# OpenRL-Lab/openrl

Measured on NVIDIA H100. Metric: env-steps/sec (collect+update), CartPole-v1 PPO, higher is better.
Workload: dtype f32 (nets, losses, Adam; the three 64x64 GEMM groups of the update run as split-fp16 wgmma MMAs with fp32 accumulation = fp32-class accuracy, the mode the 1e-4 parity tests run in), f64 (CartPole state)

## Files before the change

### include/openrl_b200.h

```cpp
#ifndef OPENRL_B200_H
#define OPENRL_B200_H

#include <stdint.h>

#ifdef __cplusplus
extern "C" {
#endif

#define ORL_ABI_VERSION 1

#define ORL_ERR_BAD_ARG 10001
#define ORL_ERR_UNSUPPORTED 10002

int orl_abi_version(void);
const char* orl_last_error(void);
int orl_device_sm_count(int* sm_count_out);

#define ORL_GAE_USE_GAE 1
#define ORL_GAE_PROPER_TIME_LIMITS 2
#define ORL_GAE_DENORM 4
#define ORL_GAE_NSTATS 8
#define ORL_GS_ADV_SUM 0
#define ORL_GS_ADV_SQSUM 1
#define ORL_GS_COUNT 2
// ... 49 lines not shown
    const float* exp_noise;
    uint64_t rng_seed;
    uint64_t rng_step_base;
    uint64_t* rng_counter;
    double* env_f64;
    uint64_t* env_u64;
    int32_t* env_i32;
    const int32_t* env_table;
    float* ep_return;
    int32_t* ep_length;
    double* episode_stats;
    int32_t head_kind;
    int32_t rng_row_offset;
} OrlRolloutArgs;
int orl_rollout(const OrlRolloutArgs* args, void* stream);

int orl_critic_values(const float* critic_params, int obs_dim, int activation_id,
                      const float* obs, float* values, long long rows, void* stream);

int orl_host_insert(const float* staged, int n_envs, int n_agents, int obs_dim, float* policy_obs_next, float* rewards,
                    float* masks_next, float* active_masks_next, void* stream);

int orl_policy_eval(const float* policy_params, int obs_dim, int n_actions, int activation_id, int head_kind,
                    const float* obs, const float* actions, const float* action_masks, float* log_probs,
                    float* entropy, long long rows, void* stream);


#define ORL_PPO_HUBER 1
#define ORL_PPO_CLIP_VALUE 2
#define ORL_PPO_VALUE_ACTIVE_MASKS 4
// ... 152 lines not shown
```

### openrl_b200/csrc/orl_fwd_tc.cu

```cuda
#include <algorithm>
#include <cstdlib>
#include <map>
#include <mutex>

#include "orl_envstep.cuh"
#include "orl_tc16.cuh"

namespace {
using namespace orl;
using namespace orl::tc;

constexpr int F_M = 128, F_NT = 256, FCW = 32;
constexpr uint32_t FPANEL_W = H * 16;
constexpr int S_LD = 68;
template <int M1, int MS>
struct FwdLayout {
    static constexpr uint32_t PANEL = M1 * 16, R1H = 0, R1L = 8 * PANEL, WH = 16 * PANEL, WL = WH + 8 * FPANEL_W, S = WL + 8 * FPANEL_W,
                              SMALL = S + MS * S_LD * 4;
};
using FLay = FwdLayout<F_M, F_M>;
constexpr uint32_t FPANEL = FLay::PANEL;
constexpr uint32_t F_SMALL_FLOATS = 8 * H + H + H + MAX_OUT * H + MAX_OUT;
constexpr uint32_t F_XCH_FLOATS = 2 * F_M * 2 + 2 * F_M * 8 + F_M * 8;
constexpr uint32_t F_SMEM = FLay::SMALL + 4 * (F_SMALL_FLOATS + F_XCH_FLOATS);

#define F_FOR_OUT(j) _Pragma("unroll") for (int j = 0; j < NOUT; ++j) if (NOUT != 8 || j < n)
#define F_ROWGROUP_SYNC()                                                      \
    do {                                                                       \
        switch (warp & 3) {                                                    \
            case 0: asm volatile("bar.sync 1, 64;" ::: "memory"); break;       \
            case 1: asm volatile("bar.sync 2, 64;" ::: "memory"); break;       \
            case 2: asm volatile("bar.sync 3, 64;" ::: "memory"); break;       \
            default: asm volatile("bar.sync 4, 64;" ::: "memory"); break;      \
        }                                                                      \
    } while (0)

template <int ACT>
__device__ __forceinline__ float f_act(float z, int activation_id) { return ACT == 1 ? fmaxf(z, 0.f) : act_fwd(z, activation_id); }

struct FwdCtx {
    uint8_t *R1h, *R1l;
    float *S, *w1t, *b1s, *b3f, *whf, *bhf, *xs, *xh, *xst;
    uint32_t aR1h, aR1l, aWh, aWl;
};

template <typename L = FLay>
__device__ __forceinline__ FwdCtx fwd_setup(uint8_t* smem, const float* __restrict__ params, int d, int n) {
    const int tid = threadIdx.x, nt = blockDim.x;
    FwdCtx c;
    c.R1h = smem + L::R1H; c.R1l = smem + L::R1L;
    uint8_t* Wh = smem + L::WH; uint8_t* Wl = smem + L::WL;
    c.S = reinterpret_cast<float*>(smem + L::S);
    c.w1t = reinterpret_cast<float*>(smem + L::SMALL);
    c.b1s = c.w1t + 8 * H; c.b3f = c.b1s + H; c.whf = c.b3f + H; c.bhf = c.whf + MAX_OUT * H;
    c.xs = c.bhf + MAX_OUT; c.xh = c.xs + 2 * F_M * 2; c.xst = c.xh + 2 * F_M * 8;
    const NetOffsets po = net_offsets(d, n);
    for (int i = tid; i < 8 * H; i += nt) { const int k = i / H, j = i % H; c.w1t[i] = (k < d) ? params[po.w1 + j * d + k] : 0.f; }
    for (int i = tid; i < H; i += nt) c.b1s[i] = params[po.b1 + i];
    for (int i = tid; i < H * 8; i += nt) {
        const int pnl = i / H, j = i % H;
        float w8[8];
#pragma unroll
        for (int c = 0; c < 8; ++c) w8[c] = params[po.w3 + j * H + 8 * pnl + c] * params[po.g1 + 8 * pnl + c];
        const uint32_t off = (uint32_t)pnl * FPANEL_W + j * 16;
        split_store8(Wh + off, Wl + off, w8, 1.0f);
    }
    for (int i = tid; i < MAX_OUT * H; i += nt) { const int j = i / H, k = i % H; c.whf[i] = (j < n) ? params[po.wh + j * H + k] * params[po.g3 + k] : 0.f; }
    for (int j = tid; j < H; j += nt) {
        float s = params[po.b3 + j];
        for (int k = 0; k < H; ++k) s = fmaf(params[po.w3 + j * H + k], params[po.be1 + k], s);
        c.b3f[j] = s;
    }
    for (int j = tid; j < MAX_OUT; j += nt) {
        float s = 0.f;
        if (j < n) { s = params[po.bh + j]; for (int k = 0; k < H; ++k) s = fmaf(params[po.wh + j * H + k], params[po.be3 + k], s); }
        c.bhf[j] = s;
    }
    fence_proxy_async();
    __syncthreads();
    c.aR1h = smem_u32(c.R1h); c.aR1l = smem_u32(c.R1l); c.aWh = smem_u32(Wh); c.aWl = smem_u32(Wl);
    return c;
}

template <int NOUT, int ACT, typename Overlap>
__device__ __forceinline__ void fwd_tile(const FwdCtx& c, const float (&x)[8], int d, int n, int activation_id,
                                         float (&out)[MAX_OUT], Overlap&& overlap) {
    const int tid = threadIdx.x, warp = tid >> 5, row = tid & 127, half = tid >> 7, cb = FCW * half;
    float n1[FCW];
#pragma unroll
    for (int q4 = 0; q4 < FCW; q4 += 4) {
        const float4 b = *reinterpret_cast<const float4*>(c.b1s + cb + q4);
        n1[q4] = b.x; n1[q4 + 1] = b.y; n1[q4 + 2] = b.z; n1[q4 + 3] = b.w;
    }
#pragma unroll
    for (int k = 0; k < 8; ++k) {
        if (k < d) {
#pragma unroll
            for (int q4 = 0; q4 < FCW; q4 += 4) {
                const float4 wv = *reinterpret_cast<const float4*>(c.w1t + k * H + cb + q4);
                n1[q4] = fmaf(x[k], wv.x, n1[q4]); n1[q4 + 1] = fmaf(x[k], wv.y, n1[q4 + 1]);
                n1[q4 + 2] = fmaf(x[k], wv.z, n1[q4 + 2]); n1[q4 + 3] = fmaf(x[k], wv.w, n1[q4 + 3]);
            }
        }
    }
    float s = 0.f, sq = 0.f;
#pragma unroll
    for (int i = 0; i < FCW; ++i) { n1[i] = f_act<ACT>(n1[i], activation_id); s += n1[i]; sq = fmaf(n1[i], n1[i], sq); }
    {
        *reinterpret_cast<float2*>(c.xs + (half * F_M + row) * 2) = make_float2(s, sq);
        F_ROWGROUP_SYNC();
        const float2 o = *reinterpret_cast<const float2*>(c.xs + ((half ^ 1) * F_M + row) * 2);
        s += o.x; sq += o.y;
    }
    const float mu1 = s * (1.f / H);
    const float rstd1 = 1.0f / sqrtf(fmaxf(sq * (1.f / H) - mu1 * mu1, 0.f) + LN_EPS);
#pragma unroll
    for (int i = 0; i < FCW; ++i) n1[i] = (n1[i] - mu1) * rstd1;
#pragma unroll
    for (int q8 = 0; q8 < FCW; q8 += 8) {
        const uint32_t off = (uint32_t)((cb + q8) >> 3) * FPANEL + row * 16;
        split_store8(c.R1h + off, c.R1l + off, n1 + q8, 1.0f);
    }
    fence_proxy_async();
    __syncthreads();
    {
        const uint64_t dK_A = desc_const(FPANEL, 128), dK_W = desc_const(FPANEL_W, 128);
        float z[32];
#pragma unroll
        for (int i = 0; i < 32; ++i) z[i] = 0.f;
        wgmma_fence();
#pragma unroll
        for (int pass = 0; pass < 3; ++pass) {
            const uint32_t aa = (pass == 0 ? c.aR1l : c.aR1h) + half * 64 * 16, bb = pass == 1 ? c.aWl : c.aWh;
#pragma unroll
            for (int kk = 0; kk < 4; ++kk)
                wgmma_f16_n64<0, 0>(z, desc_at(dK_A, aa + 2 * kk * FPANEL), desc_at(dK_W, bb + 2 * kk * FPANEL_W), (pass | kk) > 0);
        }
        wgmma_commit();
        overlap();
        wgmma_wait<0>();
        frag_store<64>(z, c.S + half * 64 * S_LD, S_LD);
    }
    __syncthreads();
    float n3[FCW];
#pragma unroll
    for (int q4 = 0; q4 < FCW; q4 += 4) {
        const float4 v = *reinterpret_cast<const float4*>(c.S + row * S_LD + cb + q4);
        n3[q4] = v.x; n3[q4 + 1] = v.y; n3[q4 + 2] = v.z; n3[q4 + 3] = v.w;
    }
    float s3 = 0.f, q3 = 0.f;
#pragma unroll
    for (int i = 0; i < FCW; ++i) { n3[i] += c.b3f[cb + i]; s3 += n3[i]; q3 = fmaf(n3[i], n3[i], q3); }
    {
        __syncwarp();
        *reinterpret_cast<float2*>(c.xs + (half * F_M + row) * 2) = make_float2(s3, q3);
        F_ROWGROUP_SYNC();
        const float2 o = *reinterpret_cast<const float2*>(c.xs + ((half ^ 1) * F_M + row) * 2);
        s3 += o.x; q3 += o.y;
    }
    const float mu3 = s3 * (1.f / H);
    const float rstd3 = 1.0f / sqrtf(fmaxf(q3 * (1.f / H) - mu3 * mu3, 0.f) + LN_EPS);
#pragma unroll
    for (int j = 0; j < MAX_OUT; ++j) out[j] = 0.f;
#pragma unroll
    for (int q4 = 0; q4 < FCW; q4 += 4) {
#pragma unroll
        for (int i = 0; i < 4; ++i) n3[q4 + i] = (n3[q4 + i] - mu3) * rstd3;
        F_FOR_OUT(j) {
            const float4 wv = *reinterpret_cast<const float4*>(c.whf + j * H + cb + q4);
            out[j] = fmaf(n3[q4], wv.x, fmaf(n3[q4 + 1], wv.y, fmaf(n3[q4 + 2], wv.z, fmaf(n3[q4 + 3], wv.w, out[j]))));
        }
    }
    {
        F_FOR_OUT(j) c.xh[(j * 2 + half) * F_M + row] = out[j];
        F_ROWGROUP_SYNC();
        F_FOR_OUT(j) {
            const float p0 = c.xh[(j * 2 + 0) * F_M + row], p1 = c.xh[(j * 2 + 1) * F_M + row];
            out[j] = (p0 + p1) + c.bhf[j];
        }
    }
}

template <int ACT>
__global__ void __launch_bounds__(F_NT, 2) critic_values_tc_kernel(const float* __restrict__ params, int d, int activation_id,
                                                                   const float* __restrict__ obs, float* __restrict__ values,
                                                                   long long rows) {
    extern __shared__ __align__(1024) uint8_t smem_f[];
    const FwdCtx c = fwd_setup(smem_f, params, d, 1);
    const int tid = threadIdx.x, warp = tid >> 5, row = tid & 127, half = tid >> 7;
    const long long n_tiles = (rows + F_M - 1) / F_M;
    for (long long tile = blockIdx.x; tile < n_tiles; tile += gridDim.x) {
        const long long r = tile * F_M + row;
        float x[8];
#pragma unroll
        for (int k = 0; k < 8; ++k) x[k] = (r < rows && k < d) ? obs[r * d + k] : 0.f;
        float out[MAX_OUT];
        fwd_tile<1, ACT>(c, x, d, 1, activation_id, out, [] {});
        if (half == 0 && r < rows) values[r] = out[0];
        F_ROWGROUP_SYNC();
    }
}

template <int ACT>
__global__ void __launch_bounds__(F_NT, 1) rollout_tc_kernel(const OrlRolloutArgs a) {
    extern __shared__ __align__(1024) uint8_t smem_f[];
    constexpr int NOUT = 5;
    const int N = a.n_envs, B = N, d = a.obs_dim, n = NOUT;
    const FwdCtx c = fwd_setup(smem_f, a.policy_params, d, n);
    const int tid = threadIdx.x, warp = tid >> 5, row = tid & 127, half = tid >> 7;
    const int e = blockIdx.x * F_M + row;
    const bool valid = e < N;
    const uint64_t rng_base = a.rng_step_base + (a.rng_counter ? *a.rng_counter : 0ull);
    float x[8];
#pragma unroll
    for (int k = 0; k < 8; ++k) x[k] = (valid && k < d) ? a.policy_obs[((size_t)a.t_begin * B + e) * d + k] : 0.f;
    {
        for (int t = a.t_begin; t < a.t_end; ++t) {
            float logit[MAX_OUT];
            float q[MAX_OUT];
            const size_t grow = (size_t)t * B + (valid ? e : 0);
            fwd_tile<NOUT, ACT>(c, x, d, n, a.activation_id, logit, [&] {
                if (half == 0 && valid && !a.deterministic)
                    action_noise(a.exp_noise, grow, n, a.rng_seed, rng_base + (uint64_t)t, (uint32_t)(e + a.rng_row_offset), q);
            });
            if (half == 0 && valid) {
                float lp;
                const int act = sample_action(logit, n, a.action_masks ? a.action_masks + grow * n : nullptr, a.deterministic != 0,
                                              [&](float (&qs)[MAX_OUT]) { for (int j = 0; j < MAX_OUT; ++j) qs[j] = q[j]; }, lp);
                a.actions[grow] = (float)act;
                a.action_log_probs[grow] = lp;
                EnvPtrs E{a.env_f64, a.env_u64, a.env_i32, a.env_table, a.env_table_len, a.rng_seed,
                          a.ep_return, a.ep_length, a.episode_stats, a.rng_row_offset};
                float ob[4], fin[4], reward; bool done;
                env_step_single(E, ORL_ENV_GRIDWORLD, e, N, act, ob, reward, done, fin);
                const size_t o1 = (size_t)(t + 1) * B + e;
                *reinterpret_cast<float4*>(a.policy_obs + o1 * 4) = make_float4(ob[0], ob[1], ob[2], ob[3]);
// ... 1 lines not shown
                a.masks[o1] = done ? 0.f : 1.f;
                a.active_masks[o1] = 1.f;
                *reinterpret_cast<float4*>(c.xst + row * 8) = make_float4(ob[0], ob[1], ob[2], ob[3]);
            }
            F_ROWGROUP_SYNC();
            if (valid) {
                const float4 o = *reinterpret_cast<const float4*>(c.xst + row * 8);
                x[0] = o.x; x[1] = o.y; x[2] = o.z; x[3] = o.w;
            }
        }
    }
}


constexpr int QCW = 16, RW_M = 64;
struct RowsCfg {
    static constexpr int R = 32, FWD = 4 * R, NT = 6 * R;
    static constexpr int MIN_CTAS = 3;
    using L = FwdLayout<RW_M, R>;
    static constexpr uint32_t XCH = L::SMALL + 4 * F_SMALL_FLOATS;
    static constexpr uint32_t XCH_F64 = XCH + 4 * (2 * MAX_OUT * R + 2 * R + 4 * R);
    static constexpr uint32_t SMEM = XCH_F64 + 8 * (2 * 2 * 4 * R + 2 * 4 * R);
    static_assert(XCH_F64 % 8 == 0, "f64 exchange area must be 8-byte aligned");
};

#define RW_FWD_SYNC() asm volatile("bar.sync 1, %0;" ::"n"(C::FWD) : "memory")
#define RW_PUBLISH_SYNC() asm volatile("bar.sync 2, %0;" ::"n"(C::NT) : "memory")

template <int ACT>
__global__ void __launch_bounds__(RowsCfg::NT, RowsCfg::MIN_CTAS) rollout_cartpole_rows_kernel(const OrlRolloutArgs a) {
    using C = RowsCfg;
    constexpr int R = C::R, NOUT = 2;
    extern __shared__ __align__(1024) uint8_t smem_f[];
    const int N = a.n_envs, B = N, n = NOUT;
    const int tid = threadIdx.x;
    for (int i = tid; i < 16 * (RW_M - R); i += C::NT) {
        const int p = i / (RW_M - R), r = R + i % (RW_M - R);
        *reinterpret_cast<uint4*>(smem_f + C::L::R1H + p * C::L::PANEL + r * 16) = make_uint4(0u, 0u, 0u, 0u);
    }
    const FwdCtx c = fwd_setup<typename C::L>(smem_f, a.policy_params, 4, n);
    float* qn = reinterpret_cast<float*>(smem_f + C::XCH);
    int* act_slot = reinterpret_cast<int*>(qn + 2 * MAX_OUT * R);
    int* termf = act_slot + 2 * R;
    double* cand = reinterpret_cast<double*>(smem_f + C::XCH_F64);
    double* srs = cand + 2 * 2 * 4 * R;
    const uint64_t rng_base = a.rng_step_base + (a.rng_counter ? *a.rng_counter : 0ull);
    uint32_t it = 0;
    if (tid >= C::FWD) {
        const int my_act = (tid - C::FWD) / R, row = (tid - C::FWD) % R;
        const int e = blockIdx.x * R + row;
        const bool valid = e < N;
        int elapsed = valid ? a.env_i32[e] : 0;
        double s[4] = {0, 0, 0, 0};
        Pcg64 g; g.state = 0; g.inc = 0;
        if (valid) {
#pragma unroll
            for (int k = 0; k < 4; ++k) s[k] = a.env_f64[(size_t)k * N + e];
            if (my_act == 0) g = pcg_load(a.env_u64, e, N);
        }
        const bool draw = my_act == 1 && valid && !a.deterministic;
        if (draw) {
            float q[MAX_OUT];
            action_noise(a.exp_noise, (size_t)a.t_begin * B + e, n, a.rng_seed, rng_base + (uint64_t)a.t_begin, (uint32_t)(e + a.rng_row_offset), q);
// ... 101 lines not shown
#pragma unroll
                    for (int kk = 0; kk < 4; ++kk)
#pragma unroll
                        for (int b = 0; b < 2; ++b)
                            wgmma_f16_n32<0, 0>(z[b], desc_at(dK_A, aa + 2 * kk * C::L::PANEL),
                                                desc_at(dK_W, bb + (nb0 + b) * 32 * 16 + 2 * kk * FPANEL_W), (pass | kk) > 0);
                }
                wgmma_commit();
                wgmma_wait<0>();
                if (16 * (warp & 3) < R) {
#pragma unroll
                    for (int b = 0; b < 2; ++b) frag_store<32>(z[b], c.S + 32 * (nb0 + b), S_LD);
                }
            }
            RW_FWD_SYNC();
            float n3[QCW];
#pragma unroll
            for (int q4 = 0; q4 < QCW; q4 += 4) {
                const float4 v = *reinterpret_cast<const float4*>(c.S + row * S_LD + cb + q4);
                n3[q4] = v.x; n3[q4 + 1] = v.y; n3[q4 + 2] = v.z; n3[q4 + 3] = v.w;
            }
            float s3 = 0.f, q3 = 0.f;
#pragma unroll
            for (int i = 0; i < QCW; ++i) { n3[i] += c.b3f[cb + i]; s3 += n3[i]; q3 = fmaf(n3[i], n3[i], q3); }
            {
                float ts = 0.f, tq = 0.f;
#pragma unroll
                for (int p = 0; p < 4; ++p) { ts += __shfl_sync(0xffffffffu, s3, qbase + p); tq += __shfl_sync(0xffffffffu, q3, qbase + p); }
                s3 = ts; q3 = tq;
            }
// ... 46 lines not shown
            if (qd == 0 && valid) {
                ret += 1.0f; len += 1;
                if (done) {
                    atomicAdd(a.episode_stats + 0, (double)ret);
                    atomicAdd(a.episode_stats + 1, (double)len);
                    atomicAdd(a.episode_stats + 2, 1.0);
                    ret = 0.f; len = 0;
                }
                const size_t o1 = (size_t)(t + 1) * B + e;
                *reinterpret_cast<float4*>(a.policy_obs + o1 * 4) = make_float4(x[0], x[1], x[2], x[3]);
                a.rewards[grow] = 1.0f;
                a.masks[o1] = done ? 0.f : 1.f;
                a.active_masks[o1] = 1.f;
            }
        }
        if (valid && qd == 0) { a.ep_return[e] = ret; a.ep_length[e] = len; }
    }
}
#undef RW_FWD_SYNC
#undef RW_PUBLISH_SYNC

template <typename K>
int prepare_kernel(K kern, uint32_t smem_bytes = F_SMEM) {
    static std::mutex mu;
    static std::map<const void*, bool> done;
    std::lock_guard<std::mutex> lock(mu);
    const void* key = reinterpret_cast<const void*>(kern);
    if (!done.count(key)) {
        int e = check_cuda(cudaFuncSetAttribute(kern, cudaFuncAttributeMaxDynamicSharedMemorySize, (int)smem_bytes), "cudaFuncSetAttribute(fwd_tc)");
        if (e) return e;
        done[key] = true;
    }
    return 0;
}

// ... 7 lines not shown
}

int launch_critic_values_tc(const float* params, int d, int activation_id, const float* obs, float* values, long long rows, cudaStream_t st) {
    const long long n_tiles = (rows + F_M - 1) / F_M;
    const int grid = (int)std::min<long long>(n_tiles, 2LL * sm_count());
    if (activation_id == 1) {
        if (int e = prepare_kernel(critic_values_tc_kernel<1>)) return e;
        critic_values_tc_kernel<1><<<grid, F_NT, F_SMEM, st>>>(params, d, activation_id, obs, values, rows);
    } else {
        if (int e = prepare_kernel(critic_values_tc_kernel<-1>)) return e;
        critic_values_tc_kernel<-1><<<grid, F_NT, F_SMEM, st>>>(params, d, activation_id, obs, values, rows);
    }
    return check_cuda(cudaGetLastError(), "critic_values_tc_kernel");
}

bool rollout_tc_eligible(const OrlRolloutArgs& a) {
    return fwd_tc_enabled() && (a.env_kind == ORL_ENV_CARTPOLE || a.env_kind == ORL_ENV_GRIDWORLD) && a.n_agents == 1 && a.obs_dim == 4 &&
           a.head_kind == ORL_HEAD_CATEGORICAL && (reinterpret_cast<uintptr_t>(a.policy_obs) & 15) == 0;
}

int launch_rollout_tc(const OrlRolloutArgs& a, cudaStream_t st) {
    const bool relu = a.activation_id == 1;
    if (a.env_kind == ORL_ENV_CARTPOLE) {
        const auto kern = relu ? rollout_cartpole_rows_kernel<1> : rollout_cartpole_rows_kernel<-1>;
        if (int e = prepare_kernel(kern, RowsCfg::SMEM)) return e;
        kern<<<(a.n_envs + RowsCfg::R - 1) / RowsCfg::R, RowsCfg::NT, RowsCfg::SMEM, st>>>(a);
        return check_cuda(cudaGetLastError(), "rollout_cartpole_rows_kernel");
    }
    const auto kern = relu ? rollout_tc_kernel<1> : rollout_tc_kernel<-1>;
    if (int e = prepare_kernel(kern)) return e;
    kern<<<(a.n_envs + F_M - 1) / F_M, F_NT, F_SMEM, st>>>(a);
    return check_cuda(cudaGetLastError(), "rollout_tc_kernel");
}

}
```

### openrl_b200/csrc/orl_rollout.cu

```cuda
#include "orl_envstep.cuh"

namespace {
using namespace orl;

constexpr int R_NT = 128;


__global__ void env_step_mpe_kernel(int N, EnvPtrs E, const float* __restrict__ actions, float* __restrict__ obs_out,
                                    float* __restrict__ critic_obs_out, float* __restrict__ rewards_out,
                                    float* __restrict__ dones_out) {
    const int e = blockIdx.x * blockDim.x + threadIdx.x;
    if (e >= N) return;
    const int acts[3] = {(int)actions[e * 3], (int)actions[e * 3 + 1], (int)actions[e * 3 + 2]};
    float ob[3][18], reward; bool done;
    env_step_mpe(E, e, N, acts, ob, reward, done);
    for (int ag = 0; ag < 3; ++ag) {
        for (int k = 0; k < 18; ++k) {
            obs_out[((size_t)e * 3 + ag) * 18 + k] = ob[ag][k];
            if (critic_obs_out) for (int dst = 0; dst < 3; ++dst) critic_obs_out[((size_t)e * 3 + dst) * 54 + ag * 18 + k] = ob[ag][k];
        }
        rewards_out[e * 3 + ag] = reward;
        dones_out[e * 3 + ag] = done ? 1.f : 0.f;
    }
}
// ... 301 lines not shown
                for (int j = 0; j < MAX_OUT; ++j) if (j < n) ent -= pr[j] * nl[j];
                logp_out[g] = lp;
                entropy_out[g] = ent;
            }
        }
        __syncthreads();
    }
}

}

namespace orl {
bool fwd_tc_enabled();
bool rollout_tc_eligible(const OrlRolloutArgs& a);
int launch_rollout_tc(const OrlRolloutArgs& a, cudaStream_t st);
int launch_critic_values_tc(const float* params, int d, int activation_id, const float* obs, float* values, long long rows, cudaStream_t st);
}

extern "C" int orl_env_reset(int env_kind, int n_envs, int n_agents, double* env_f64, uint64_t* env_u64,
                             int32_t* env_i32, const int32_t* env_table, int env_table_len, uint64_t rng_seed,
                             float* policy_obs_out, float* critic_obs_out, void* stream) {
    ORL_CHECK_ARG(n_envs > 0 && n_agents > 0, "n_envs/n_agents");
    ORL_CHECK_ARG(policy_obs_out, "policy_obs_out");
    if (env_kind == ORL_ENV_CARTPOLE) ORL_CHECK_ARG(env_f64 && env_u64 && env_i32 && n_agents == 1, "cartpole state");
    else if (env_kind == ORL_ENV_GRIDWORLD) ORL_CHECK_ARG(env_i32 && n_agents == 1, "gridworld state");
    else if (env_kind == ORL_ENV_MPE_SPREAD) ORL_CHECK_ARG(env_f64 && env_u64 && env_i32 && n_agents == 3, "simple_spread state");
    else { orl::set_last_error("orl_env_reset: unsupported env_kind %d", env_kind); return ORL_ERR_UNSUPPORTED; }
    cudaStream_t st = reinterpret_cast<cudaStream_t>(stream);
    env_reset_kernel<<<(n_envs + 127) / 128, 128, 0, st>>>(env_kind, n_envs, env_f64, env_u64, env_i32, env_table,
                                                          env_table_len, rng_seed, policy_obs_out, critic_obs_out);
// ... 15 lines not shown
            n_envs, Em, actions, obs_out, final_obs_out, rewards_out, dones_out);
        ORL_LAUNCH_CHECK("env_step_mpe_kernel");
        return 0;
    }
    ORL_CHECK_ARG(n_agents == 1, "n_agents");
    if (env_kind == ORL_ENV_CARTPOLE) ORL_CHECK_ARG(env_f64 && env_u64 && env_i32, "cartpole state");
    else if (env_kind == ORL_ENV_GRIDWORLD) ORL_CHECK_ARG(env_i32, "gridworld state");
    else { orl::set_last_error("orl_env_step: unsupported env_kind %d", env_kind); return ORL_ERR_UNSUPPORTED; }
    EnvPtrs E{env_f64, env_u64, env_i32, env_table, env_table_len, rng_seed, ep_return, ep_length, episode_stats};
    env_step_kernel<<<(n_envs + 127) / 128, 128, 0, reinterpret_cast<cudaStream_t>(stream)>>>(
        env_kind, n_envs, E, actions, obs_out, rewards_out, dones_out, final_obs_out);
    ORL_LAUNCH_CHECK("env_step_kernel");
    return 0;
}

extern "C" int orl_rollout(const OrlRolloutArgs* args, void* stream) {
    ORL_CHECK_ARG(args, "args");
    const OrlRolloutArgs& a = *args;
    ORL_CHECK_ARG(a.n_envs > 0 && a.n_agents > 0 && a.n_agents <= 32, "n_envs / n_agents");
    ORL_CHECK_ARG(a.obs_dim > 0 && a.obs_dim <= 64, "obs_dim must be in 1..64");
    ORL_CHECK_ARG(a.n_actions > 0 && a.n_actions <= orl::MAX_OUT, "n_actions must be in 1..8");
    ORL_CHECK_ARG(a.t_begin >= 0 && a.t_begin < a.t_end && a.t_end <= a.episode_length, "step range");
    ORL_CHECK_ARG(a.activation_id >= 0 && a.activation_id <= 3, "activation_id");
    ORL_CHECK_ARG(a.policy_params && a.policy_obs && a.actions && a.action_log_probs, "null buffer");
    ORL_CHECK_ARG(a.head_kind == ORL_HEAD_CATEGORICAL || (a.head_kind == ORL_HEAD_GAUSSIAN && a.env_kind == ORL_ENV_NONE),
                  "Gaussian heads act on host-stepped envs (ORL_ENV_NONE)");
    if (a.env_kind == ORL_ENV_NONE) {
        ORL_CHECK_ARG(a.t_end == a.t_begin + 1, "ORL_ENV_NONE acts for one step per call");
    } else if (a.env_kind == ORL_ENV_CARTPOLE) {
        ORL_CHECK_ARG(a.n_agents == 1 && a.obs_dim == 4 && a.n_actions == 2, "CartPole shapes");
        ORL_CHECK_ARG(a.env_f64 && a.env_u64 && a.env_i32 && a.rewards && a.masks && a.active_masks && a.ep_return &&
                          a.ep_length && a.episode_stats, "CartPole state buffers");
    } else if (a.env_kind == ORL_ENV_GRIDWORLD) {
        ORL_CHECK_ARG(a.n_agents == 1 && a.obs_dim == 4 && a.n_actions == 5, "GridWorld shapes");
        ORL_CHECK_ARG(a.env_i32 && a.rewards && a.masks && a.active_masks && a.ep_return && a.ep_length &&
                          a.episode_stats, "GridWorld state buffers");
    } else if (a.env_kind == ORL_ENV_MPE_SPREAD) {
        ORL_CHECK_ARG(a.n_agents == 3 && a.obs_dim == 18 && a.critic_obs_dim == 54 && a.n_actions == 5, "simple_spread shapes");
        ORL_CHECK_ARG(a.env_f64 && a.env_u64 && a.env_i32 && a.rewards && a.masks && a.active_masks && a.ep_return &&
                          a.ep_length && a.episode_stats && a.critic_obs, "simple_spread state buffers");
    } else {
        orl::set_last_error("orl_rollout: unsupported env_kind %d", a.env_kind);
        return ORL_ERR_UNSUPPORTED;
    }
    cudaStream_t st = reinterpret_cast<cudaStream_t>(stream);
    if (orl::rollout_tc_eligible(a)) {
        if (int e = orl::launch_rollout_tc(a, st)) return e;
        return orl::bump_rng_counter(a.rng_counter, a.t_end - a.t_begin, st);
    }
    const long long B = (long long)a.n_envs * a.n_agents;
    const long long want = 4LL * orl::sm_count();
    int rm = 32;
    if (B / 32 < want) rm = 16;
    if (B / 16 < want) rm = 8;
    while (rm < a.n_agents) rm *= 2;
    const int envs_per_cta = rm / a.n_agents;
    const int grid = (a.n_envs + envs_per_cta - 1) / envs_per_cta;
    const int ldx = orl::pad4(a.obs_dim) + 4;
    const size_t smem = sizeof(float) * (orl::smem_weights_floats(a.obs_dim, false) + rm * ldx + 2 * rm * orl::LDA + rm);
// ... 11 lines not shown
    do {                                                                                 \
        if (rm == 8) ORL_LAUNCH_ROLLOUT(8, EK);                                          \
        else if (rm == 16) ORL_LAUNCH_ROLLOUT(16, EK);                                   \
        else ORL_LAUNCH_ROLLOUT(32, EK);                                                 \
    } while (0)
    switch (a.env_kind) {
        case ORL_ENV_NONE: ORL_LAUNCH_ROLLOUT_RM(ORL_ENV_NONE); break;
        case ORL_ENV_CARTPOLE: ORL_LAUNCH_ROLLOUT_RM(ORL_ENV_CARTPOLE); break;
        case ORL_ENV_GRIDWORLD: ORL_LAUNCH_ROLLOUT_RM(ORL_ENV_GRIDWORLD); break;
        default: ORL_LAUNCH_ROLLOUT_RM(ORL_ENV_MPE_SPREAD); break;
    }
    ORL_LAUNCH_CHECK("rollout_kernel");
    return orl::bump_rng_counter(a.rng_counter, a.t_end - a.t_begin, st);
}

extern "C" int orl_critic_values(const float* critic_params, int obs_dim, int activation_id, const float* obs,
                                 float* values, long long rows, void* stream) {
    ORL_CHECK_ARG(critic_params && obs && values, "null buffer");
    ORL_CHECK_ARG(obs_dim > 0 && obs_dim <= 64, "obs_dim must be in 1..64");
    ORL_CHECK_ARG(rows > 0, "rows");
    ORL_CHECK_ARG(activation_id >= 0 && activation_id <= 3, "activation_id");
    if (orl::fwd_tc_enabled() && obs_dim <= 8)
        return orl::launch_critic_values_tc(critic_params, obs_dim, activation_id, obs, values, rows, reinterpret_cast<cudaStream_t>(stream));
    const int ldx = orl::pad4(obs_dim) + 4;
    const size_t smem = sizeof(float) * (orl::smem_weights_floats(obs_dim, false) + C_M * ldx + 2 * C_M * orl::LDA);
    static bool attr_set = false;
    if (!attr_set) {
        int e = orl::check_cuda(cudaFuncSetAttribute(critic_values_kernel, cudaFuncAttributeMaxDynamicSharedMemorySize, 200 * 1024),
                                "cudaFuncSetAttribute(critic_values)");
        if (e) return e;
// ... 57 lines not shown
```

### openrl_b200/drivers/onpolicy_driver.py

```python
import numpy as np
import torch

from .. import lib


class OnPolicyDriver:
    def __init__(self, config, trainer, buffer, agent, rank=0, world_size=1, client=None, logger=None, callback=None):
        cfg = config["cfg"]
        self.cfg = cfg
        self.trainer, self.buffer, self.agent = trainer, buffer, agent
        self.envs = config["envs"]
        self.device = config["device"]
        self.num_agents = config["num_agents"]
        self.rank, self.world_size = rank, world_size
        self.logger, self.callback = logger, callback
        self.num_env_steps = cfg.num_env_steps
        self.episode_length = cfg.episode_length
        self.n_rollout_threads = cfg.n_rollout_threads
        self.learner_n_rollout_threads = cfg.learner_n_rollout_threads
        self.use_linear_lr_decay = cfg.use_linear_lr_decay
        self.log_interval = cfg.log_interval
        self.episode = 0
        self.total_num_steps = 0
        self._lib = lib.load()
        self._global_step = 0
        self.rng_counter = torch.zeros(1, dtype=torch.int64, device=self.device)
        self.gpu_launches = 0
        self.h2d_bytes = 0
        self.d2h_bytes = 0
        self.phase_events = None
        self.recurrent = bool(cfg.use_recurrent_policy or getattr(cfg, "use_naive_recurrent_policy", False))
        if self.recurrent and self.envs.kind == lib.ENV_NONE and getattr(cfg, "use_joint_action_loss", False):
            raise NotImplementedError("use_joint_action_loss (JRPO) is built for simple_spread on the device (3 agents, agent-0 "
                                      "critic); host-stepped envs take the per-agent recurrent update")

    def run(self):
        episodes = int(self.num_env_steps) // self.episode_length // self.learner_n_rollout_threads
        self.episodes = episodes
        self.reset_and_buffer_init()
        for episode in range(episodes):
            if self.cfg.log_each_episode and self.logger is not None:
                self.logger.info("Episode: {}/{}".format(episode, episodes))
# ... 225 lines not shown
    def _launch_steps(self, t_begin, t_end, noise):
        s = lib.current_stream()
        if self.recurrent:
            lib.check(self._lib.orl_rnn_rollout(self._rnn_args(t_begin, t_end, noise), s), "orl_rnn_rollout")
            self.gpu_launches += 2
        elif self.envs.kind == lib.ENV_GRIDWORLD_2P:
            if getattr(self.trainer, "share", False) or noise is not None:
                raise NotImplementedError("the self-play rollout is built for the two-net MLP policy with device sampling")
            sp = self.envs.selfplay_args(self._rollout_args(t_begin, t_end, None))
            lib.check(self._lib.orl_selfplay_rollout(sp, s), "orl_selfplay_rollout")
            self.gpu_launches += 2
        elif getattr(self.trainer, "share", False):
            lib.check(self._lib.orl_share_rollout(self._rollout_args(t_begin, t_end, noise), s), "orl_share_rollout")
            self.gpu_launches += 2
        else:
            lib.check(self._lib.orl_rollout(self._rollout_args(t_begin, t_end, noise), s), "orl_rollout")
            self.gpu_launches += 2

    def _draw_noise(self):
        d = self.buffer.data
        B, n = d.n_rollout_threads * d.num_agents, d.n_actions
        host = torch.empty(self.episode_length, B, n, dtype=torch.float32, pin_memory=True)
        gaussian = self.trainer.algo_module.models["policy"].head_kind == lib.HEAD_GAUSSIAN
        for t in range(self.episode_length):
            if gaussian:
                host[t].normal_()
            else:
                host[t].exponential_(1)
        self.h2d_bytes += host.numel() * 4
        return host.to(self.device, non_blocking=True)

    def _rollout_launch(self):
# ... 125 lines not shown
                    if step + 1 < T:
                        env.group_fetch_actions(g, lo, hi, self._act_rows(step + 1, lo, hi))
                self.agent.num_time_steps += N
        self._host_steps_base += T
        return True

    @torch.no_grad()
    def compute_returns(self):
        d = self.buffer.data
        cri = self.trainer.algo_module.models["critic"]
        rows = (self.episode_length + 1) * d.n_rollout_threads * d.num_agents
        if self.recurrent:
            with self._phase("critic"):
                lib.check(self._lib.orl_rnn_critic(self._rnn_args(0, self.episode_length, None), lib.current_stream()),
                          "orl_rnn_critic")
            with self._phase("gae"):
                self.buffer.compute_returns(None, self.trainer.algo_module.get_critic_value_normalizer())
            self.gpu_launches += 2
            return
        with self._phase("critic"):
            if getattr(self.trainer, "share", False):
                lib.check(self._lib.orl_share_values(lib.ptr(cri.flat_params), cri.obs_dim, cri.n_actions, cri.activation_id,
                                                     lib.ptr(d.critic_obs), lib.ptr(d.value_preds), rows, lib.current_stream()),
                          "orl_share_values")
            else:
                lib.check(self._lib.orl_critic_values(lib.ptr(cri.flat_params), cri.obs_dim, cri.activation_id,
                                                      lib.ptr(d.critic_obs), lib.ptr(d.value_preds), rows,
                                                      lib.current_stream()), "orl_critic_values")
        with self._phase("gae"):
            self.buffer.compute_returns(None, self.trainer.algo_module.get_critic_value_normalizer())
        self.gpu_launches += 2
```

### openrl_b200/lib.py

```python
import ctypes
import os
import re

HERE = os.path.dirname(os.path.abspath(__file__))
LIB_PATH = os.path.join(HERE, "csrc", "libopenrl_b200.so")
HEADER = os.path.join(os.path.dirname(HERE), "include", "openrl_b200.h")


class OrlLibraryError(RuntimeError):
    pass


class OrlError(RuntimeError):
    pass


_c = ctypes
_P = _c.c_void_p
_I = _c.c_int
_D = _c.c_double
_F = _c.c_float
_L = _c.c_longlong

_SIGNATURES = {
# ... 107 lines not shown
    ]


class OrlPeerArgs(ctypes.Structure):
    _fields_ = [
        ("peer_buffers", _P), ("local_buffer", _P), ("epochs", _P), ("error_flag", _P), ("summed", _P),
        ("world", _c.c_int32), ("rank", _c.c_int32), ("timeout_ms", _c.c_int32), ("reserved", _c.c_int32),
    ]


PEER_MAX_WORLD = 16

_SIGNATURES.update({
    "orl_env_reset": [_I, _I, _I, _P, _P, _P, _P, _I, _c.c_uint64, _P, _P, _P],
    "orl_rollout": [_c.POINTER(OrlRolloutArgs), _P],
    "orl_env_step": [_I, _I, _I, _P, _P, _P, _P, _I, _c.c_uint64, _P, _P, _P, _P, _P, _P, _P, _P, _P],
    "orl_critic_values": [_P, _I, _I, _P, _P, _L, _P],
    "orl_selfplay_reset": [_c.POINTER(OrlSelfPlayArgs), _P, _P],
    "orl_selfplay_rollout": [_c.POINTER(OrlSelfPlayArgs), _P],
    "orl_share_param_count": [_I, _I],
    "orl_share_tape_width": [],
    "orl_share_workspace_floats": [_L, _I, _I],
    "orl_share_rollout": [_c.POINTER(OrlRolloutArgs), _P],
    "orl_share_values": [_P, _I, _I, _I, _P, _P, _L, _P],
    "orl_share_fwdbwd": [_c.POINTER(OrlPpoArgs), _P],
    "orl_share_apply": [_c.POINTER(OrlPpoArgs), _P],
    "orl_host_insert": [_P, _I, _I, _I, _P, _P, _P, _P, _P],
    "orl_policy_eval": [_P, _I, _I, _I, _I, _P, _P, _P, _P, _P, _L, _P],
    "orl_ppo_stride": [_I, _I, _I],
    "orl_ppo_grads_stride": [_I, _I, _I],
# ... 39 lines not shown


_SIGNATURES.update({
    "orl_rnn_act_rows": [_c.POINTER(OrlRnnArgs), _P],
    "orl_host_insert_rnn": [_P, _I, _I, _I, _P, _P, _P, _P, _P, _P],
    "orl_rnn_param_count": [_I, _I],
    "orl_rnn_tape_width": [],
    "orl_rnn_workspace_floats": [_c.c_int64, _I],
    "orl_rnn_rollout": [_c.POINTER(OrlRnnArgs), _P],
    "orl_rnn_critic": [_c.POINTER(OrlRnnArgs), _P],
    "orl_rnn_fwdbwd": [_c.POINTER(OrlRnnArgs), _P],
    "orl_rnn_apply": [_c.POINTER(OrlRnnArgs), _P],
})

ENV_NONE, ENV_CARTPOLE, ENV_GRIDWORLD, ENV_MPE_SPREAD, ENV_GRIDWORLD_2P = 0, 1, 2, 3, 4
SP_RANDOM, SP_LAST = 0, 1
HEAD_CATEGORICAL, HEAD_GAUSSIAN = 0, 1
GAE_USE_GAE, GAE_PROPER_TIME_LIMITS, GAE_DENORM = 1, 2, 4
PPO_HUBER, PPO_CLIP_VALUE, PPO_VALUE_ACTIVE_MASKS, PPO_POLICY_ACTIVE_MASKS = 1, 2, 4, 8
PPO_VALUENORM, PPO_ADV_NORMALIZE, PPO_MAX_GRAD_NORM, PPO_TENSORCORE = 16, 32, 64, 128
PPO_TF32 = PPO_TENSORCORE
PPO_A2C, PPO_DUAL_CLIP = 256, 512
PPO_JOINT_ACTION = 1024
```

Measured before the change: 230.1 million.

## Fuse critic value computation into CartPole rollout kernel via extra warpgroup

Adds a variant of the CartPole rollout kernel with an extra 128-thread warpgroup that runs the critic forward pass on observations two timesteps at a time, synchronised with the policy warps through named barriers. The driver uses this path when critic obs equals policy obs and skips the separate critic_values launch. This removes a kernel launch and a second pass over the observation buffer. In exchange the fused kernel uses more threads and shared memory (MIN_CTAS drops from 3 to 2), adds barrier coupling that may stall the policy/env loop, and lowers occupancy.

New measurement: 234.2 million (median of 6 runs). +1.8%, better.

```diff
diff --git a/include/openrl_b200.h b/include/openrl_b200.h
--- a/include/openrl_b200.h
+++ b/include/openrl_b200.h
@@ -87,6 +87,8 @@
     int32_t rng_row_offset;
 } OrlRolloutArgs;
 int orl_rollout(const OrlRolloutArgs* args, void* stream);
+
+int orl_rollout_values(const OrlRolloutArgs* args, const float* critic_params, float* value_preds, void* stream);
 
 int orl_critic_values(const float* critic_params, int obs_dim, int activation_id,
                       const float* obs, float* values, long long rows, void* stream);
diff --git a/openrl_b200/csrc/orl_fwd_tc.cu b/openrl_b200/csrc/orl_fwd_tc.cu
--- a/openrl_b200/csrc/orl_fwd_tc.cu
+++ b/openrl_b200/csrc/orl_fwd_tc.cu
@@ -13,27 +13,33 @@
 constexpr int F_M = 128, F_NT = 256, FCW = 32;
 constexpr uint32_t FPANEL_W = H * 16;
 constexpr int S_LD = 68;
+constexpr uint32_t F_SMALL_FLOATS = 8 * H + H + H + MAX_OUT * H + MAX_OUT;
 template <int M1, int MS>
 struct FwdLayout {
+    static constexpr int M = M1;
     static constexpr uint32_t PANEL = M1 * 16, R1H = 0, R1L = 8 * PANEL, WH = 16 * PANEL, WL = WH + 8 * FPANEL_W, S = WL + 8 * FPANEL_W,
-                              SMALL = S + MS * S_LD * 4;
+                              SMALL = S + MS * S_LD * 4, XST = SMALL + 4 * (F_SMALL_FLOATS + 2 * M1 * 2 + 2 * M1 * 8),
+                              END = XST + 4 * M1 * 8;
 };
 using FLay = FwdLayout<F_M, F_M>;
-constexpr uint32_t FPANEL = FLay::PANEL;
-constexpr uint32_t F_SMALL_FLOATS = 8 * H + H + H + MAX_OUT * H + MAX_OUT;
-constexpr uint32_t F_XCH_FLOATS = 2 * F_M * 2 + 2 * F_M * 8 + F_M * 8;
-constexpr uint32_t F_SMEM = FLay::SMALL + 4 * (F_SMALL_FLOATS + F_XCH_FLOATS);
+constexpr uint32_t F_SMEM = FLay::END;
 
 #define F_FOR_OUT(j) _Pragma("unroll") for (int j = 0; j < NOUT; ++j) if (NOUT != 8 || j < n)
-#define F_ROWGROUP_SYNC()                                                      \
-    do {                                                                       \
-        switch (warp & 3) {                                                    \
-            case 0: asm volatile("bar.sync 1, 64;" ::: "memory"); break;       \
-            case 1: asm volatile("bar.sync 2, 64;" ::: "memory"); break;       \
-            case 2: asm volatile("bar.sync 3, 64;" ::: "memory"); break;       \
-            default: asm volatile("bar.sync 4, 64;" ::: "memory"); break;      \
-        }                                                                      \
-    } while (0)
+
+struct CtaTileSync {
+    static constexpr int M = 128;
+    __device__ __forceinline__ static int tid() { return threadIdx.x; }
+    __device__ __forceinline__ static void tile() { __syncthreads(); }
+    __device__ __forceinline__ static void rows(int warp) {
+        switch (warp & 3) {
+            case 0: asm volatile("bar.sync 1, 64;" ::: "memory"); break;
+            case 1: asm volatile("bar.sync 2, 64;" ::: "memory"); break;
+            case 2: asm volatile("bar.sync 3, 64;" ::: "memory"); break;
+            default: asm volatile("bar.sync 4, 64;" ::: "memory"); break;
+        }
+    }
+};
+#define F_ROWGROUP_SYNC() CtaTileSync::rows(warp)
 
 template <int ACT>
 __device__ __forceinline__ float f_act(float z, int activation_id) { return ACT == 1 ? fmaxf(z, 0.f) : act_fwd(z, activation_id); }
@@ -53,7 +59,7 @@
     c.S = reinterpret_cast<float*>(smem + L::S);
     c.w1t = reinterpret_cast<float*>(smem + L::SMALL);
     c.b1s = c.w1t + 8 * H; c.b3f = c.b1s + H; c.whf = c.b3f + H; c.bhf = c.whf + MAX_OUT * H;
-    c.xs = c.bhf + MAX_OUT; c.xh = c.xs + 2 * F_M * 2; c.xst = c.xh + 2 * F_M * 8;
+    c.xs = c.bhf + MAX_OUT; c.xh = c.xs + 2 * L::M * 2; c.xst = c.xh + 2 * L::M * 8;
     const NetOffsets po = net_offsets(d, n);
     for (int i = tid; i < 8 * H; i += nt) { const int k = i / H, j = i % H; c.w1t[i] = (k < d) ? params[po.w1 + j * d + k] : 0.f; }
     for (int i = tid; i < H; i += nt) c.b1s[i] = params[po.b1 + i];
@@ -82,10 +88,13 @@
     return c;
 }
 
-template <int NOUT, int ACT, typename Overlap>
+template <typename Sync, int NOUT, int ACT, typename Overlap>
 __device__ __forceinline__ void fwd_tile(const FwdCtx& c, const float (&x)[8], int d, int n, int activation_id,
                                          float (&out)[MAX_OUT], Overlap&& overlap) {
-    const int tid = threadIdx.x, warp = tid >> 5, row = tid & 127, half = tid >> 7, cb = FCW * half;
+    constexpr int M = Sync::M;
+    constexpr uint32_t FPANEL = M * 16;
+    const int tid = Sync::tid() & (2 * M - 1), warp = tid >> 5, row = tid & (M - 1), half = tid / M, cb = FCW * half;
+    const int wg = tid >> 7;
     float n1[FCW];
 #pragma unroll
     for (int q4 = 0; q4 < FCW; q4 += 4) {
@@ -107,9 +116,9 @@
 #pragma unroll
     for (int i = 0; i < FCW; ++i) { n1[i] = f_act<ACT>(n1[i], activation_id); s += n1[i]; sq = fmaf(n1[i], n1[i], sq); }
     {
-        *reinterpret_cast<float2*>(c.xs + (half * F_M + row) * 2) = make_float2(s, sq);
-        F_ROWGROUP_SYNC();
-        const float2 o = *reinterpret_cast<const float2*>(c.xs + ((half ^ 1) * F_M + row) * 2);
+        *reinterpret_cast<float2*>(c.xs + (half * M + row) * 2) = make_float2(s, sq);
+        Sync::rows(warp);
+        const float2 o = *reinterpret_cast<const float2*>(c.xs + ((half ^ 1) * M + row) * 2);
         s += o.x; sq += o.y;
     }
     const float mu1 = s * (1.f / H);
@@ -122,7 +131,7 @@
         split_store8(c.R1h + off, c.R1l + off, n1 + q8, 1.0f);
     }
     fence_proxy_async();
-    __syncthreads();
+    Sync::tile();
     {
         const uint64_t dK_A = desc_const(FPANEL, 128), dK_W = desc_const(FPANEL_W, 128);
         float z[32];
@@ -131,7 +140,7 @@
         wgmma_fence();
 #pragma unroll
         for (int pass = 0; pass < 3; ++pass) {
-            const uint32_t aa = (pass == 0 ? c.aR1l : c.aR1h) + half * 64 * 16, bb = pass == 1 ? c.aWl : c.aWh;
+            const uint32_t aa = (pass == 0 ? c.aR1l : c.aR1h) + wg * 64 * 16, bb = pass == 1 ? c.aWl : c.aWh;
 #pragma unroll
             for (int kk = 0; kk < 4; ++kk)
                 wgmma_f16_n64<0, 0>(z, desc_at(dK_A, aa + 2 * kk * FPANEL), desc_at(dK_W, bb + 2 * kk * FPANEL_W), (pass | kk) > 0);
@@ -139,9 +148,9 @@
         wgmma_commit();
         overlap();
         wgmma_wait<0>();
-        frag_store<64>(z, c.S + half * 64 * S_LD, S_LD);
-    }
-    __syncthreads();
+        frag_store<64>(z, c.S + wg * 64 * S_LD, S_LD);
+    }
+    Sync::tile();
     float n3[FCW];
 #pragma unroll
     for (int q4 = 0; q4 < FCW; q4 += 4) {
@@ -153,9 +162,9 @@
     for (int i = 0; i < FCW; ++i) { n3[i] += c.b3f[cb + i]; s3 += n3[i]; q3 = fmaf(n3[i], n3[i], q3); }
     {
         __syncwarp();
-        *reinterpret_cast<float2*>(c.xs + (half * F_M + row) * 2) = make_float2(s3, q3);
-        F_ROWGROUP_SYNC();
-        const float2 o = *reinterpret_cast<const float2*>(c.xs + ((half ^ 1) * F_M + row) * 2);
+        *reinterpret_cast<float2*>(c.xs + (half * M + row) * 2) = make_float2(s3, q3);
+        Sync::rows(warp);
+        const float2 o = *reinterpret_cast<const float2*>(c.xs + ((half ^ 1) * M + row) * 2);
         s3 += o.x; q3 += o.y;
     }
     const float mu3 = s3 * (1.f / H);
@@ -172,10 +181,10 @@
         }
     }
     {
-        F_FOR_OUT(j) c.xh[(j * 2 + half) * F_M + row] = out[j];
-        F_ROWGROUP_SYNC();
+        F_FOR_OUT(j) c.xh[(j * 2 + half) * M + row] = out[j];
+        Sync::rows(warp);
         F_FOR_OUT(j) {
-            const float p0 = c.xh[(j * 2 + 0) * F_M + row], p1 = c.xh[(j * 2 + 1) * F_M + row];
+            const float p0 = c.xh[(j * 2 + 0) * M + row], p1 = c.xh[(j * 2 + 1) * M + row];
             out[j] = (p0 + p1) + c.bhf[j];
         }
     }
@@ -195,7 +204,7 @@
 #pragma unroll
         for (int k = 0; k < 8; ++k) x[k] = (r < rows && k < d) ? obs[r * d + k] : 0.f;
         float out[MAX_OUT];
-        fwd_tile<1, ACT>(c, x, d, 1, activation_id, out, [] {});
+        fwd_tile<CtaTileSync, 1, ACT>(c, x, d, 1, activation_id, out, [] {});
         if (half == 0 && r < rows) values[r] = out[0];
         F_ROWGROUP_SYNC();
     }
@@ -219,7 +228,7 @@
             float logit[MAX_OUT];
             float q[MAX_OUT];
             const size_t grow = (size_t)t * B + (valid ? e : 0);
-            fwd_tile<NOUT, ACT>(c, x, d, n, a.activation_id, logit, [&] {
+            fwd_tile<CtaTileSync, NOUT, ACT>(c, x, d, n, a.activation_id, logit, [&] {
                 if (half == 0 && valid && !a.deterministic)
                     action_noise(a.exp_noise, grow, n, a.rng_seed, rng_base + (uint64_t)t, (uint32_t)(e + a.rng_row_offset), q);
             });
@@ -251,31 +260,49 @@
 
 
 constexpr int QCW = 16, RW_M = 64;
+template <bool VALUES>
 struct RowsCfg {
-    static constexpr int R = 32, FWD = 4 * R, NT = 6 * R;
-    static constexpr int MIN_CTAS = 3;
+    static constexpr int R = 32, FWD = 4 * R, PE = 6 * R, CR = VALUES ? 128 : 0, NT = PE + CR;
+    static constexpr int MIN_CTAS = VALUES ? 2 : 3;
     using L = FwdLayout<RW_M, R>;
     static constexpr uint32_t XCH = L::SMALL + 4 * F_SMALL_FLOATS;
     static constexpr uint32_t XCH_F64 = XCH + 4 * (2 * MAX_OUT * R + 2 * R + 4 * R);
-    static constexpr uint32_t SMEM = XCH_F64 + 8 * (2 * 2 * 4 * R + 2 * 4 * R);
+    static constexpr uint32_t POLICY_END = XCH_F64 + 8 * (2 * 2 * 4 * R + 2 * 4 * R);
     static_assert(XCH_F64 % 8 == 0, "f64 exchange area must be 8-byte aligned");
+    using CL = FwdLayout<2 * R, 2 * R>;
+    static constexpr uint32_t CBASE = (POLICY_END + 1023u) & ~1023u;
+    static constexpr uint32_t SMEM = VALUES ? CBASE + CL::XST : POLICY_END;
 };
 
 #define RW_FWD_SYNC() asm volatile("bar.sync 1, %0;" ::"n"(C::FWD) : "memory")
-#define RW_PUBLISH_SYNC() asm volatile("bar.sync 2, %0;" ::"n"(C::NT) : "memory")
-
-template <int ACT>
-__global__ void __launch_bounds__(RowsCfg::NT, RowsCfg::MIN_CTAS) rollout_cartpole_rows_kernel(const OrlRolloutArgs a) {
-    using C = RowsCfg;
+#define RW_PUBLISH_SYNC() asm volatile("bar.sync 2, %0;" ::"n"(C::PE) : "memory")
+#define RW_JOINT_SYNC() asm volatile("bar.sync 3, %0;" ::"n"(C::FWD + C::CR) : "memory")
+
+struct RowsCriticSync {
+    static constexpr int M = 64;
+    __device__ __forceinline__ static int tid() { int t; asm volatile("mov.u32 %0, %%tid.x;" : "=r"(t)); return t; }
+    __device__ __forceinline__ static void tile() { asm volatile("bar.sync 4, 128;" ::: "memory"); }
+    __device__ __forceinline__ static void rows(int warp) {
+        if (warp & 1) asm volatile("bar.sync 6, 64;" ::: "memory");
+        else asm volatile("bar.sync 5, 64;" ::: "memory");
+    }
+};
+
+template <int ACT, bool VALUES>
+__global__ void __launch_bounds__(RowsCfg<VALUES>::NT, RowsCfg<VALUES>::MIN_CTAS)
+    rollout_cartpole_rows_kernel(const OrlRolloutArgs a, const float* __restrict__ critic_params, float* __restrict__ values) {
+    using C = RowsCfg<VALUES>;
     constexpr int R = C::R, NOUT = 2;
     extern __shared__ __align__(1024) uint8_t smem_f[];
     const int N = a.n_envs, B = N, n = NOUT;
-    const int tid = threadIdx.x;
-    for (int i = tid; i < 16 * (RW_M - R); i += C::NT) {
+    for (int i = threadIdx.x; i < 16 * (RW_M - R); i += C::NT) {
         const int p = i / (RW_M - R), r = R + i % (RW_M - R);
         *reinterpret_cast<uint4*>(smem_f + C::L::R1H + p * C::L::PANEL + r * 16) = make_uint4(0u, 0u, 0u, 0u);
     }
     const FwdCtx c = fwd_setup<typename C::L>(smem_f, a.policy_params, 4, n);
+    FwdCtx cc{};
+    if constexpr (VALUES) cc = fwd_setup<typename C::CL>(smem_f + C::CBASE, critic_params, 4, 1);
+    const int tid = threadIdx.x - C::CR;
     float* qn = reinterpret_cast<float*>(smem_f + C::XCH);
     int* act_slot = reinterpret_cast<int*>(qn + 2 * MAX_OUT * R);
     int* termf = act_slot + 2 * R;
@@ -283,7 +310,25 @@
     double* srs = cand + 2 * 2 * 4 * R;
     const uint64_t rng_base = a.rng_step_base + (a.rng_counter ? *a.rng_counter : 0ull);
     uint32_t it = 0;
-    if (tid >= C::FWD) {
+    if (VALUES && threadIdx.x < C::CR) {
+        for (int s0 = 0; s0 <= a.t_end - a.t_begin; s0 += 2) {
+            RW_JOINT_SYNC();
+            const int row = RowsCriticSync::tid() & (RowsCriticSync::M - 1), s = s0 + row / R;
+            const int e = blockIdx.x * R + row % R;
+            const bool live = e < N && a.t_begin + s <= a.t_end;
+            const size_t grow = (size_t)(a.t_begin + s) * B + e;
+            float x[8];
+#pragma unroll
+            for (int k = 0; k < 8; ++k) x[k] = 0.f;
+            if (live) {
+                const float4 o = *reinterpret_cast<const float4*>(a.policy_obs + grow * 4);
+                x[0] = o.x; x[1] = o.y; x[2] = o.z; x[3] = o.w;
+            }
+            float out[MAX_OUT];
+            fwd_tile<RowsCriticSync, 1, ACT>(cc, x, 4, 1, a.activation_id, out, [] {});
+            if (threadIdx.x < RowsCriticSync::M && live) values[grow] = out[0];
+        }
+    } else if (tid >= C::FWD) {
         const int my_act = (tid - C::FWD) / R, row = (tid - C::FWD) % R;
         const int e = blockIdx.x * R + row;
         const bool valid = e < N;
@@ -415,6 +460,7 @@
                 }
             }
             RW_FWD_SYNC();
+            if (VALUES && (it & 1u)) RW_JOINT_SYNC();
             float n3[QCW];
 #pragma unroll
             for (int q4 = 0; q4 < QCW; q4 += 4) {
@@ -491,11 +537,13 @@
                 a.active_masks[o1] = 1.f;
             }
         }
+        if constexpr (VALUES) RW_JOINT_SYNC();
         if (valid && qd == 0) { a.ep_return[e] = ret; a.ep_length[e] = len; }
     }
 }
 #undef RW_FWD_SYNC
 #undef RW_PUBLISH_SYNC
+#undef RW_JOINT_SYNC
 
 template <typename K>
 int prepare_kernel(K kern, uint32_t smem_bytes = F_SMEM) {
@@ -533,6 +581,15 @@
     return check_cuda(cudaGetLastError(), "critic_values_tc_kernel");
 }
 
+template <bool VALUES>
+int launch_rollout_cartpole(const OrlRolloutArgs& a, const float* critic_params, float* values, cudaStream_t st) {
+    using C = RowsCfg<VALUES>;
+    const auto kern = a.activation_id == 1 ? rollout_cartpole_rows_kernel<1, VALUES> : rollout_cartpole_rows_kernel<-1, VALUES>;
+    if (int e = prepare_kernel(kern, C::SMEM)) return e;
+    kern<<<(a.n_envs + C::R - 1) / C::R, C::NT, C::SMEM, st>>>(a, critic_params, values);
+    return check_cuda(cudaGetLastError(), "rollout_cartpole_rows_kernel");
+}
+
 bool rollout_tc_eligible(const OrlRolloutArgs& a) {
     return fwd_tc_enabled() && (a.env_kind == ORL_ENV_CARTPOLE || a.env_kind == ORL_ENV_GRIDWORLD) && a.n_agents == 1 && a.obs_dim == 4 &&
            a.head_kind == ORL_HEAD_CATEGORICAL && (reinterpret_cast<uintptr_t>(a.policy_obs) & 15) == 0;
@@ -540,16 +597,15 @@
 
 int launch_rollout_tc(const OrlRolloutArgs& a, cudaStream_t st) {
     const bool relu = a.activation_id == 1;
-    if (a.env_kind == ORL_ENV_CARTPOLE) {
-        const auto kern = relu ? rollout_cartpole_rows_kernel<1> : rollout_cartpole_rows_kernel<-1>;
-        if (int e = prepare_kernel(kern, RowsCfg::SMEM)) return e;
-        kern<<<(a.n_envs + RowsCfg::R - 1) / RowsCfg::R, RowsCfg::NT, RowsCfg::SMEM, st>>>(a);
-        return check_cuda(cudaGetLastError(), "rollout_cartpole_rows_kernel");
-    }
+    if (a.env_kind == ORL_ENV_CARTPOLE) return launch_rollout_cartpole<false>(a, nullptr, nullptr, st);
     const auto kern = relu ? rollout_tc_kernel<1> : rollout_tc_kernel<-1>;
     if (int e = prepare_kernel(kern)) return e;
     kern<<<(a.n_envs + F_M - 1) / F_M, F_NT, F_SMEM, st>>>(a);
     return check_cuda(cudaGetLastError(), "rollout_tc_kernel");
 }
 
-}
+int launch_rollout_values_tc(const OrlRolloutArgs& a, const float* critic_params, float* values, cudaStream_t st) {
+    return launch_rollout_cartpole<true>(a, critic_params, values, st);
+}
+
+}
diff --git a/openrl_b200/csrc/orl_rollout.cu b/openrl_b200/csrc/orl_rollout.cu
--- a/openrl_b200/csrc/orl_rollout.cu
+++ b/openrl_b200/csrc/orl_rollout.cu
@@ -339,6 +339,7 @@
 bool fwd_tc_enabled();
 bool rollout_tc_eligible(const OrlRolloutArgs& a);
 int launch_rollout_tc(const OrlRolloutArgs& a, cudaStream_t st);
+int launch_rollout_values_tc(const OrlRolloutArgs& a, const float* critic_params, float* values, cudaStream_t st);
 int launch_critic_values_tc(const float* params, int d, int activation_id, const float* obs, float* values, long long rows, cudaStream_t st);
 }
 
@@ -384,7 +385,8 @@
     return 0;
 }
 
-extern "C" int orl_rollout(const OrlRolloutArgs* args, void* stream) {
+namespace {
+int check_rollout_args(const OrlRolloutArgs* args) {
     ORL_CHECK_ARG(args, "args");
     const OrlRolloutArgs& a = *args;
     ORL_CHECK_ARG(a.n_envs > 0 && a.n_agents > 0 && a.n_agents <= 32, "n_envs / n_agents");
@@ -413,6 +415,13 @@
         orl::set_last_error("orl_rollout: unsupported env_kind %d", a.env_kind);
         return ORL_ERR_UNSUPPORTED;
     }
+    return 0;
+}
+}
+
+extern "C" int orl_rollout(const OrlRolloutArgs* args, void* stream) {
+    if (int e = check_rollout_args(args)) return e;
+    const OrlRolloutArgs& a = *args;
     cudaStream_t st = reinterpret_cast<cudaStream_t>(stream);
     if (orl::rollout_tc_eligible(a)) {
         if (int e = orl::launch_rollout_tc(a, st)) return e;
@@ -454,6 +463,19 @@
     return orl::bump_rng_counter(a.rng_counter, a.t_end - a.t_begin, st);
 }
 
+extern "C" int orl_rollout_values(const OrlRolloutArgs* args, const float* critic_params, float* value_preds, void* stream) {
+    if (int e = check_rollout_args(args)) return e;
+    const OrlRolloutArgs& a = *args;
+    ORL_CHECK_ARG(critic_params && value_preds, "null buffer");
+    if (a.env_kind != ORL_ENV_CARTPOLE || a.critic_obs_dim != 0 || !orl::rollout_tc_eligible(a)) {
+        orl::set_last_error("orl_rollout_values: only the tensor-core CartPole rollout with critic obs == policy obs computes values");
+        return ORL_ERR_UNSUPPORTED;
+    }
+    cudaStream_t st = reinterpret_cast<cudaStream_t>(stream);
+    if (int e = orl::launch_rollout_values_tc(a, critic_params, value_preds, st)) return e;
+    return orl::bump_rng_counter(a.rng_counter, a.t_end - a.t_begin, st);
+}
+
 extern "C" int orl_critic_values(const float* critic_params, int obs_dim, int activation_id, const float* obs,
                                  float* values, long long rows, void* stream) {
     ORL_CHECK_ARG(critic_params && obs && values, "null buffer");
diff --git a/openrl_b200/drivers/onpolicy_driver.py b/openrl_b200/drivers/onpolicy_driver.py
--- a/openrl_b200/drivers/onpolicy_driver.py
+++ b/openrl_b200/drivers/onpolicy_driver.py
@@ -26,6 +26,7 @@
         self._global_step = 0
         self.rng_counter = torch.zeros(1, dtype=torch.int64, device=self.device)
         self.gpu_launches = 0
+        self.values_in_rollout = False
         self.h2d_bytes = 0
         self.d2h_bytes = 0
         self.phase_events = None
@@ -281,8 +282,19 @@
             lib.check(self._lib.orl_share_rollout(self._rollout_args(t_begin, t_end, noise), s), "orl_share_rollout")
             self.gpu_launches += 2
         else:
-            lib.check(self._lib.orl_rollout(self._rollout_args(t_begin, t_end, noise), s), "orl_rollout")
+            a = self._rollout_args(t_begin, t_end, noise)
+            d = self.buffer.data
+            if self.envs.kind == lib.ENV_CARTPOLE and d.critic_obs is d.policy_obs:
+                cri = self.trainer.algo_module.models["critic"]
+                rc = self._lib.orl_rollout_values(a, lib.ptr(cri.flat_params), lib.ptr(d.value_preds), s)
+                if rc != lib.ERR_UNSUPPORTED:
+                    lib.check(rc, "orl_rollout_values")
+                    self.values_in_rollout = True
+                    self.gpu_launches += 2
+                    return
+            lib.check(self._lib.orl_rollout(a, s), "orl_rollout")
             self.gpu_launches += 2
+        self.values_in_rollout = False
 
     def _draw_noise(self):
         d = self.buffer.data
@@ -438,19 +450,18 @@
             with self._phase("critic"):
                 lib.check(self._lib.orl_rnn_critic(self._rnn_args(0, self.episode_length, None), lib.current_stream()),
                           "orl_rnn_critic")
-            with self._phase("gae"):
-                self.buffer.compute_returns(None, self.trainer.algo_module.get_critic_value_normalizer())
-            self.gpu_launches += 2
-            return
-        with self._phase("critic"):
-            if getattr(self.trainer, "share", False):
-                lib.check(self._lib.orl_share_values(lib.ptr(cri.flat_params), cri.obs_dim, cri.n_actions, cri.activation_id,
-                                                     lib.ptr(d.critic_obs), lib.ptr(d.value_preds), rows, lib.current_stream()),
-                          "orl_share_values")
-            else:
-                lib.check(self._lib.orl_critic_values(lib.ptr(cri.flat_params), cri.obs_dim, cri.activation_id,
-                                                      lib.ptr(d.critic_obs), lib.ptr(d.value_preds), rows,
-                                                      lib.current_stream()), "orl_critic_values")
+            self.gpu_launches += 1
+        elif not self.values_in_rollout:
+            with self._phase("critic"):
+                if getattr(self.trainer, "share", False):
+                    lib.check(self._lib.orl_share_values(lib.ptr(cri.flat_params), cri.obs_dim, cri.n_actions, cri.activation_id,
+                                                         lib.ptr(d.critic_obs), lib.ptr(d.value_preds), rows, lib.current_stream()),
+                              "orl_share_values")
+                else:
+                    lib.check(self._lib.orl_critic_values(lib.ptr(cri.flat_params), cri.obs_dim, cri.activation_id,
+                                                          lib.ptr(d.critic_obs), lib.ptr(d.value_preds), rows,
+                                                          lib.current_stream()), "orl_critic_values")
+            self.gpu_launches += 1
         with self._phase("gae"):
             self.buffer.compute_returns(None, self.trainer.algo_module.get_critic_value_normalizer())
-        self.gpu_launches += 2
+        self.gpu_launches += 1
diff --git a/openrl_b200/lib.py b/openrl_b200/lib.py
--- a/openrl_b200/lib.py
+++ b/openrl_b200/lib.py
@@ -145,6 +145,7 @@
 _SIGNATURES.update({
     "orl_env_reset": [_I, _I, _I, _P, _P, _P, _P, _I, _c.c_uint64, _P, _P, _P],
     "orl_rollout": [_c.POINTER(OrlRolloutArgs), _P],
+    "orl_rollout_values": [_c.POINTER(OrlRolloutArgs), _P, _P, _P],
     "orl_env_step": [_I, _I, _I, _P, _P, _P, _P, _I, _c.c_uint64, _P, _P, _P, _P, _P, _P, _P, _P, _P],
     "orl_critic_values": [_P, _I, _I, _P, _P, _L, _P],
     "orl_selfplay_reset": [_c.POINTER(OrlSelfPlayArgs), _P, _P],
@@ -214,6 +215,7 @@
 })
 
 ENV_NONE, ENV_CARTPOLE, ENV_GRIDWORLD, ENV_MPE_SPREAD, ENV_GRIDWORLD_2P = 0, 1, 2, 3, 4
+ERR_BAD_ARG, ERR_UNSUPPORTED = 10001, 10002
 SP_RANDOM, SP_LAST = 0, 1
 HEAD_CATEGORICAL, HEAD_GAUSSIAN = 0, 1
 GAE_USE_GAE, GAE_PROPER_TIME_LIMITS, GAE_DENORM = 1, 2, 4
```
